# Hevagog/as-cops-and-thieves

Measured on AMD Instinct MI355X. Metric: env-steps/sec (whole node) at 4096 parallel envs, 2v1 agents, 64-ray sensors, higher is better.
Workload: dtype f64; 1 GPU; 2 cops vs 1 thieves, labyrinth map (30 hull walls / 119 planes), 4096 envs per GPU, 64 rays/agent, dt=1/60, max_step_count=400, Philox random actions, auto-reset; envs_per_gpu=4096, rays=64, agents=3, map=labyrinth, parallelism=env-sharded x1, no data-path collective, episodes_reset_per_gpu=32768, burn_in_steps=600

## Files before the change

as_cops_and_thieves_amd/_native.py:

```python
from __future__ import annotations

import ctypes as C
import os
import subprocess
from pathlib import Path

from .config import C_FIELDS_F64, C_FIELDS_I32

PKG = Path(__file__).resolve().parent
ROOT = PKG.parent
LIB_PATH = PKG / "libcat_sim.so"
if os.environ.get("CAT_SIM_LIB"):
    LIB_PATH = Path(os.environ["CAT_SIM_LIB"]).resolve()
SRC = PKG / "csrc" / "cat_sim.hip"


def sources():
    return [SRC, *sorted((PKG / "csrc").glob("cat_sim_*.h")), ROOT / "include" / "cat_sim.h"]
HIPCC_FLAGS = ["--offload-arch=gfx950", "-O3", "-ffp-contract=off", "-fPIC", "-shared"]

OUT_FIELDS = ("obs_distance", "obs_type", "hit_shape", "shared_distance", "shared_type",
              "team_positions", "reward", "terminated", "truncated", "winner")
STATE_FIELDS = ("pos", "vel", "vbias", "tc", "leaf_bb", "wall_shape", "wall_age", "wall_jn",
                "pair_age", "pair_jn", "step_count", "reset_count")
# ... 100 lines not shown
    L.cat_grid_free_host.restype = None
    L.cat_map_wall_bb_depth_host.argtypes = [vp, C.c_size_t, C.c_double]
    L.cat_map_wall_bb_depth_host.restype = i32
    if hasattr(L, "cat_bbtree_host"):
        L.cat_bbtree_host.argtypes = [vp, C.c_size_t, vp, vp, i32, vp, vp]
        L.cat_bbtree_host.restype = i32
    if hasattr(L, "cat_plan_describe_host"):
        L.cat_plan_describe_host.argtypes = [vp, vp, vp, vp, i32, vp, C.c_char_p, C.c_size_t]
        L.cat_plan_describe_host.restype = i32
    if hasattr(L, "cat_debug_tree_counts"):
        L.cat_debug_tree_counts.argtypes = [vp, i32]
        L.cat_debug_tree_counts.restype = i32
    if hasattr(L, "cat_radius_thresholds_host"):
        L.cat_radius_thresholds_host.argtypes = [C.c_double, C.c_double, C.c_double, vp]
        L.cat_radius_thresholds_host.restype = i32
    if hasattr(L, "cat_reward_arith_host"):
        L.cat_reward_arith_host.argtypes = [vp, vp, vp]
        L.cat_reward_arith_host.restype = i32
        L.cat_reward_arith_max.argtypes = [vp]
        L.cat_reward_arith_max.restype = i32
        L.cat_debug_reward_table.argtypes = [vp, vp, vp]
        L.cat_debug_reward_table.restype = i32
    for name in ("cat_create", "cat_destroy", "cat_reset", "cat_reset_done", "cat_step", "cat_step_fused", "cat_rollout_fused", "cat_step_repeat", "cat_get_state",
                 "cat_set_state", "cat_random_actions", "cat_set_seed", "cat_device_errors", "cat_arm_kernel_timing", "cat_num_agents", "cat_num_shapes", "cat_selftest_arith", "cat_debug_grid_lookup"):
        getattr(L, name).restype = i32
    _lib = L
    return L


EXPORTED_SYMBOLS = ("cat_abi_version", "cat_one_tick_kernel", "cat_rollout_kernel", "cat_chunks_per_unit", "cat_last_error", "cat_create", "cat_destroy", "cat_reset",
                    "cat_reset_done", "cat_step", "cat_step_fused", "cat_rollout_fused", "cat_step_repeat", "cat_get_state", "cat_set_state", "cat_random_actions",
                    "cat_set_seed", "cat_device_errors", "cat_arm_kernel_timing", "cat_num_agents", "cat_num_shapes", "cat_selftest_arith", "cat_debug_grid_lookup",
                    "cat_grid_build_host", "cat_grid_lookup_host", "cat_grid_bytes_host", "cat_grid_free_host", "cat_map_wall_bb_depth_host",
                    "cat_bbtree_host", "cat_reward_arith_host", "cat_reward_arith_max", "cat_debug_reward_table", "cat_bind_final_positions",
                    "cat_plan_describe_host", "cat_radius_thresholds_host")
```

as_cops_and_thieves_amd/csrc/cat_sim.hip:

```cpp
#include <hip/hip_runtime.h>
#include <hip/hip_ext.h>

#include <cfloat>
#include <cmath>
#include <cstdarg>
#include <cstdint>
#include <cstdio>
#include <cstdlib>
#include <cstring>
#include <algorithm>
#include <atomic>
#include <thread>
#include <type_traits>
#include <sched.h>
#include <string>
#include <vector>

#include "cat_sim.h"

namespace {
#include "cat_sim_common.h"
#include "cat_sim_reward.h"
#include "cat_sim_geometry.h"
#include "cat_sim_fan.h"
#include "cat_sim_physics.h"
#include "cat_sim_scheduler.h"
}

#include "cat_sim_grid.h"
#include "cat_sim_radius.h"
#include "cat_sim_plan.h"
#include "cat_sim_host.h"
```

as_cops_and_thieves_amd/csrc/cat_sim_common.h:

```cpp

constexpr int kMaxWaves = 16;
constexpr int kLanes = 64;
constexpr int kK = CAT_WALL_CACHE;
constexpr int kBB = 6;
constexpr int kPairF = 20;
constexpr unsigned kBlobMagic = 0x31544143u;

struct MapDesc {
    int S, P, A, n_regions;
    int f64_off;
    int i32_off;
    float cmax;
    int PP;
};

struct GridDesc {
    double x0, y0, inv_cell;
    int nx, ny;
    int off_base, ent_base;
    int coff_base, cent_base;
    int crow_base, span;
    int row_base, span_tick;
};

// ... 27 lines not shown
    char *state;
    int rec_bytes, hot_bytes;
    int maxE, ang_ok, row_words, row_id_bits, row_cnt_mul;
    float ang0, inv_step;
    int lds_map_bytes, lds_env_bytes, lds_union_bytes;
    int wpb;
    int lds_pool_off, pool_mask;
    int grp_rays;
    int item_cap;
    unsigned pool_magic; int pool_shift;
    const double *tree_bb;
    const int *tree_link;
    const int *tree_root;
    int lds_racc_off;
    int lds_o16_off;
};

struct DynDims {
    static constexpr bool kFixed = false;
    static constexpr bool kTree = false;
    static __device__ __forceinline__ int A(const Params &p) { return p.A; }
    static __device__ __forceinline__ int R(const Params &p) { return p.R; }
    static __device__ __forceinline__ int n_cops(const Params &p) { return p.n_cops; }
    static __device__ __forceinline__ int NP(const Params &p) { return p.NP; }
    static __device__ __forceinline__ int rec_bytes(const Params &p) { return p.rec_bytes; }
    static __device__ __forceinline__ int hot_bytes(const Params &p) { return p.hot_bytes; }
};
template <int TA, int TR, int TC> struct FixDims {
    static constexpr bool kFixed = true;
    static constexpr bool kTree = false;
// ... 54 lines not shown
        prev = t;
    }
    __device__ void flush(int lane) { if (lane < 24 && acc[lane]) atomicAdd(&g_phase_cycles[lane], acc[lane]); }
};
#define PHASE(pc, id) (pc).mark(id)
#ifdef CAT_EVENT_COUNTS
#define QCOUNT(id) do { const unsigned long long m_ = __ballot(true); if ((int)__builtin_ctzll(m_) == (int)(threadIdx.x % 64)) { \
    atomicAdd(&g_phase_cycles[id], 1ull); atomicAdd(&g_phase_cycles[(id) + 1], (unsigned long long)__popcll(m_)); } } while (0)
#else
#define QCOUNT(id) do {} while (0)
#endif
#else
#define QCOUNT(id) do {} while (0)
struct PhaseClock { __device__ __forceinline__ void flush(int) {} };
#define PHASE(pc, id) do {} while (0)
#endif

struct LaunchArgs {
    cat_outputs out;
    const int *actions;
    union {
        const unsigned char *mask;
        unsigned short *final_pos;
    };
    const double *positions;
    int use_done_mask;
    int auto_reset;
    unsigned long long synth_tick;
    int T;
    int repeat;
// ... 152 lines not shown
```

as_cops_and_thieves_amd/csrc/cat_sim_fan.h:

```cpp
constexpr int kFeatNear = 63;
constexpr int kItemCap = 128;
constexpr int kPassJ = 8;
constexpr int kFanBytes = 2 * kItemCap * 8 + kItemCap * 2 + kPassJ * kLanes * 2;
constexpr int kGroupRays = 256;

__device__ __forceinline__ void poly_query_feat(const Lds &L, float cmax, bool wall, int sh, double r, double cx, double cy, double ax, double ay,
                                                double bx, double by, double r2, double &alpha, int &feat)
{
    const int fc = wall ? L.fc[sh] : 0, first = fc & 0xFFFF, count = fc >> 16;
    const double rsum = r + r2, rr = rsum * rsum;
    const float axf = (float)ax, ayf = (float)ay;
    const float dxf = (float)(bx - ax), dyf = (float)(by - ay);
    const float len2 = dxf * dxf + dyf * dyf, len = sqrtf(len2);
    const float e1 = 1e-6f * (fabsf(axf) + fabsf(ayf) + cmax + 512.0f);
    const float thr = ((float)rsum + 0.01f) * len * 1.00001f + 0.25f + 64.0f * e1;
    const float s_lo = -((float)rsum + 1.0f) * len, s_hi = len2 + ((float)rsum + 1.0f) * len;
    const bool bevels = rsum > 0.0;
    unsigned pm = 0u, vm = wall ? 0u : 1u;
    const double *pl0 = L.planes + 8 * first;
    {
        typedef float f32x2 __attribute__((ext_vector_type(2)));
        const float *q = L.p32 + kPairF * (wall ? L.fp[sh] : 0);
        const f32x2 ax2 = {axf, axf}, ay2 = {ayf, ayf}, dx2 = {dxf, dxf}, dy2 = {dyf, dyf};
        const f32x2 len3 = {3.0f * len, 3.0f * len}, four = {4.0f, 4.0f};
// ... 1005 lines not shown
```

as_cops_and_thieves_amd/csrc/cat_sim_geometry.h:

```cpp
__device__ __forceinline__ double bb_segment_query(const double *bb, double ax, double ay, double dx,
                                                   double dy, double idx, double idy)
{
    const double2 lo = *reinterpret_cast<const double2 *>(bb);
    const double2 hi = *reinterpret_cast<const double2 *>(bb + 2);
    double tmin = -INFINITY, tmax = INFINITY;
    if (dx == 0.0) {
        if (ax < lo.x || hi.x < ax) return INFINITY;
    } else {
        double t1 = (lo.x - ax) * idx, t2 = (hi.x - ax) * idx;
        tmin = CAT_FMAX(tmin, CAT_FMIN(t1, t2));
        tmax = CAT_FMIN(tmax, CAT_FMAX(t1, t2));
    }
    if (dy == 0.0) {
        if (ay < lo.y || hi.y < ay) return INFINITY;
    } else {
        double t1 = (lo.y - ay) * idy, t2 = (hi.y - ay) * idy;
        tmin = CAT_FMAX(tmin, CAT_FMIN(t1, t2));
        tmax = CAT_FMIN(tmax, CAT_FMAX(t1, t2));
    }
    if (tmin <= tmax && 0.0 <= tmax && tmin <= 1.0) return CAT_FMAX(tmin, 0.0);
    return INFINITY;
}

struct SegInfo { int hit; double alpha, px, py; };

__device__ __forceinline__ void circle_segment_query(double cx, double cy, double r1, double ax, double ay,
                                                     double bx, double by, double r2, SegInfo &info)
{
    double dax = ax - cx, day = ay - cy, dbx = bx - cx, dby = by - cy;
    double rsum = r1 + r2;
    double dada = dax * dax + day * day, dadb = dax * dbx + day * dby, dbdb = dbx * dbx + dby * dby;
    double qa = dada - 2.0 * dadb + dbdb;
    double qb = dadb - dada;
    double det = qb * qb - qa * (dada - rsum * rsum);
// ... 99 lines not shown
```

as_cops_and_thieves_amd/csrc/cat_sim_host.h:

```cpp
struct Part {
    GridHost grid;
    std::vector<int> map_ids;
    Params p;
    Params *dev_p = nullptr;
    Prologue pro;
    int n_blocks = 0, wpb = 0, n_envs = 0;
    size_t lds_bytes = 0;
    bool pool_step = false;
    KernelChoice kernels;
};

struct cat_sim {
    std::vector<Part> parts;
    int device;
    hipStream_t side = nullptr;
    hipEvent_t ev_fork = nullptr, ev_join = nullptr;
    hipEvent_t t_start = nullptr, t_stop = nullptr;
    uint16_t *final_pos = nullptr;
    std::vector<MapDesc> maps;
    std::vector<void *> allocs;
    std::string one_tick_name, rollout_name;
    char err[256];
};

// ... 378 lines not shown
        return CAT_ERR_NO_DEVICE;
    }
    if (hipSetDevice(device) != hipSuccess) return CAT_ERR_NO_DEVICE;
    hipLaunchKernelGGL(selftest_kernel, dim3((n + 255) / 256), dim3(256), 0, static_cast<hipStream_t>(stream), op, a, b, out, n);
    return hipGetLastError() == hipSuccess ? CAT_OK : CAT_ERR_HIP;
}

extern "C" int cat_radius_thresholds_host(double term_radius, double agent_radius, double ray_radius, double *out2)
{
    if (!out2) return CAT_ERR_BAD_ARG;
    out2[0] = radius_lt_threshold(term_radius);
    out2[1] = radius_le_threshold(agent_radius, ray_radius);
    return CAT_OK;
}

extern "C" int cat_reward_arith_host(const float *cop_lut, const float *thief_lut, float *out)
{
    if (out)
        for (int i = 0; i < 2 * 32768; i++) out[i] = (float)ra_host_f16_to_f64(reward_arith_f16(i < 32768, (unsigned)i & 0x7FFFu));
    return cop_lut && thief_lut ? reward_arith_scan(cop_lut, thief_lut) : -1;
}

extern "C" int cat_reward_arith_max(const cat_sim *s)
{
    if (!s) return CAT_ERR_BAD_ARG;
    std::vector<float> lut(2 * 32768);
    if (hipSetDevice(s->device) != hipSuccess) return CAT_ERR_NO_DEVICE;
    if (hipMemcpy(lut.data(), s->parts[0].p.cop_lut, 32768 * sizeof(float), hipMemcpyDeviceToHost) != hipSuccess ||
        hipMemcpy(lut.data() + 32768, s->parts[0].p.thief_lut, 32768 * sizeof(float), hipMemcpyDeviceToHost) != hipSuccess) return CAT_ERR_HIP;
    return reward_arith_scan(lut.data(), lut.data() + 32768);
// ... 10 lines not shown
```

as_cops_and_thieves_amd/csrc/cat_sim_physics.h:

```cpp

__device__ __forceinline__ int circle_poly_contact(const Lds &L, int sh, double rp, double cx, double cy, double rc, int lane,
                                   double &nx, double &ny, double &p1x, double &p1y, double &p2x, double &p2y)
{
    const int fc = uni(L.fc[sh]), first = fc & 0xFFFF, count = fc >> 16;
    double sep = -INFINITY, dd = INFINITY, tt = 0.0, ppx = 0.0, ppy = 0.0;
    if (lane < count) {
        const double *pl = L.planes + 8 * (first + lane);
        sep = pl[0] * (cx - pl[2]) + pl[1] * (cy - pl[3]);
    }
    if (__ballot(sep > rc + rp + 1e-9) != 0ull) return 0;
    if (lane < count) {
        const int i = lane;
        const double *pl = L.planes + 8 * (first + i);
        const double *pv = L.planes + 8 * (first + (i - 1 + count) % count);
        double ax_ = pl[2] - cx, ay_ = pl[3] - cy, bx_ = pv[2] - cx, by_ = pv[3] - cy;
        double dx = bx_ - ax_, dy = by_ - ay_;
        double t = -fmin2(fmax2((dx * (ax_ + bx_) + dy * (ay_ + by_)) / (dx * dx + dy * dy), -1.0), 1.0);
        double ht = 0.5 * t;
        ppx = ax_ * (0.5 - ht) + bx_ * (0.5 + ht); ppy = ay_ * (0.5 - ht) + by_ * (0.5 + ht);
        dd = ppx * ppx + ppy * ppy;
        tt = t;
    }
    const bool inside = __ballot(sep > 0.0) == 0ull;
    int best = 0, sepi = 0;
// ... 254 lines not shown
            else L.wag[lane] = a;
        }
    }
    if (lane < D::NP(p)) {
        const int page = L.pag[lane];
        if (page >= 0 && !((seen_p >> lane) & 1u)) {
            const int a = page + 1;
            if (a >= p.persistence) { L.pag[lane] = -1; L.pjn[lane] = 0.0; }
            else L.pag[lane] = a;
        }
    }
    wave_sync();
    PHASE(pc, 15);
    if (nc == 0) return;
    wave_sync();
    const double m_inv = 1.0 / p.mass;
    const int q = lane;
    const bool own = q < nc;
    {
        int ka = -1, kb = -1;
        if (own) { const int *ci = reinterpret_cast<const int *>(L.conf + kConD * q + 12); ka = ci[0]; kb = ci[1]; }
        bool reg = __ballot(kb >= 0) == 0ull;
        int k0 = 0, kn = 0;
        for (int i = 0; reg && i < A; i++) {
            const unsigned long long mk = __ballot(ka == i);
            if (mk == 0ull) continue;
            const int n_i = __popcll(mk), f_i = __builtin_ctzll(mk);
            if (n_i > kSolveReg || mk != (((1ull << n_i) - 1ull) << f_i)) { reg = false; break; }
            if (lane == i) { k0 = f_i; kn = n_i; }
        }
        if (reg) { solve_walls_reg(L, p, lane, k0, kn, m_inv); wave_sync(); return; }
// ... 59 lines not shown
```

as_cops_and_thieves_amd/csrc/cat_sim_plan.h:

```cpp

struct RecLayout {
    int A, NPs;
    constexpr explicit RecLayout(int a) : A(a), NPs(a * (a - 1) / 2 > 0 ? a * (a - 1) / 2 : 1) {}
    constexpr int pos() const { return 0; }
    constexpr int vel() const { return 16 * A; }
    constexpr int vbias() const { return 32 * A; }
    constexpr int tc() const { return 48 * A; }
    constexpr int leaf_bb() const { return 64 * A; }
    constexpr int step_count() const { return 96 * A; }
    constexpr int reset_count() const { return 96 * A + 4; }
    constexpr int hot_bytes() const { return 96 * A + 16; }
    constexpr int wall_jn() const { return hot_bytes(); }
    constexpr int pair_jn() const { return hot_bytes() + A * kK * 8; }
    constexpr int wall_shape() const { return hot_bytes() + (A * kK + NPs) * 8; }
    constexpr int wall_age() const { return wall_shape() + A * kK * 4; }
    constexpr int pair_age() const { return wall_shape() + 2 * A * kK * 4; }
    constexpr int cold_bytes() const { return ((A * kK + NPs) * 8 + (2 * A * kK + NPs) * 4 + 15) / 16 * 16; }
    constexpr int rec_bytes() const { return hot_bytes() + cold_bytes(); }
};

struct LdsSizes {
    int map, env, uni;
    int racc;
    int o16;
// ... 486 lines not shown
        if (slot_map_ids) plan.slot[e] = slot_map_ids[e];
        if (plan.slot[e] < 0 || plan.slot[e] >= n_maps) PLAN_FAIL(CAT_ERR_BAD_SLOT_MAP, "slot_map_ids[%d]=%d out of range", e, plan.slot[e]);
    }
    std::vector<GridHost> map_grid;
    plan_map_grids(cfg, tab, plan, map_grid);
    Params &base = plan.base;
    memset(&base, 0, sizeof base);
    base.N = N; base.A = A; base.n_cops = cfg->n_cops; base.R = cfg->n_rays; base.max_step = cfg->max_step_count;
    base.iterations = cfg->iterations; base.persistence = cfg->persistence; base.gate = cfg->bbtree_gate;
    base.NP = A * (A - 1) / 2;
    base.env_id_offset = cfg->env_id_offset; base.seed = cfg->seed;
    base.dt = cfg->dt; base.bias_coef = cfg->bias_coef; base.slop = cfg->slop; base.ray_length = cfg->ray_length;
    base.ray_radius = cfg->ray_radius; base.rc = cfg->agent_radius; base.mass = cfg->agent_mass; base.impulse = cfg->impulse;
    base.max_speed = cfg->max_speed; base.term_radius = cfg->termination_radius; base.wall_r = cfg->wall_radius;
    base.term_d2 = radius_lt_threshold(base.term_radius); base.near_d2 = radius_le_threshold(base.rc, base.ray_radius);
    base.hot_bytes = RecLayout(A).hot_bytes();
    base.rec_bytes = RecLayout(A).rec_bytes();
    if (base.hot_bytes > kLanes * 16) PLAN_FAIL(CAT_ERR_BAD_CONFIG, "state record of %d bytes exceeds the kernels' register staging", base.hot_bytes);
    split_parts(cfg, map_grid, plan);
    plan_initial_records(cfg, plan);
    {
        const double two_pi = 6.283185307179586;
        const double a0 = atan2(tab->ray_dy[0], tab->ray_dx[0]);
        const double step = two_pi / base.R;
        bool ok = base.R >= 4;
        for (int k = 0; k < base.R && ok; k++) {
            double d = atan2(tab->ray_dy[k], tab->ray_dx[k]) - (a0 + k * step);
            d -= two_pi * floor(d / two_pi + 0.5);
            if (fabs(d) > 1e-6) ok = false;
        }
// ... 124 lines not shown
```

as_cops_and_thieves_amd/csrc/cat_sim_scheduler.h:

```cpp
template <class D>
__device__ __forceinline__ Lds carve(const Params &p, char *smem, const MapDesc &md, int slot, int wave)
{
    Lds L;
    const int S = md.S, P = md.P, W = p.wpb;
    L.bb = reinterpret_cast<const double *>(smem);
    L.planes = L.bb + kBB * S;
    L.p32 = reinterpret_cast<const float *>(L.planes + 8 * P);
    L.fc = reinterpret_cast<const int *>(L.planes + geo_rest_doubles(md));
    L.fp = L.fc + S;
    L.rayd = reinterpret_cast<const double *>(smem + p.lds_map_bytes - 16 * D::R(p));
    L.ctrl = reinterpret_cast<int *>(smem + p.lds_map_bytes);
    char *w = smem + p.lds_map_bytes + ctrl_bytes(W) + slot * p.lds_env_bytes;
    const int A = D::A(p), R = D::R(p), NPs = D::NP(p) > 0 ? D::NP(p) : 1;
    L.rec = w;
    double *d = reinterpret_cast<double *>(w);
    L.pos = d; d += 2 * A; L.vel = d; d += 2 * A; L.vb = d; d += 2 * A; L.tc = d; d += 2 * A;
    L.leaf = d; d += 4 * A;
    L.cnt = reinterpret_cast<int *>(d);
    d = reinterpret_cast<double *>(w + D::hot_bytes(p));
    L.wjn = d; d += A * kK; L.pjn = d; d += NPs;
    {
        int *ri = reinterpret_cast<int *>(d);
        L.wsh = ri; ri += A * kK; L.wag = ri; ri += A * kK; L.pag = ri;
    }
// ... 370 lines not shown
                                          int env, int row_t, int lane, int act_pref, unsigned long long synth_tick, int n_fan, PhaseClock &pc)
{
    int captured, timeout, step;
    SetupRow row;
    {
        const Params &p = *(const Params *)launder(pk);
        const int S = md.S, A = D::A(p);
        row = setup_row(L.pos, p, gd, lane, A);
        step = uni(L.cnt[0]) + 1;
        captured = termination_captured<D>(L, p, S, lane);
        timeout = (!captured && step >= p.max_step) ? 1 : 0;
        copy_snapshot(L, A, lane);

        if (lane < A) {
            const int i = lane;
            const double m_inv = 1.0 / p.mass;
            int act;
            if (la.actions) act = act_pref;
            else { unsigned rnd[4]; philox_env(p, env, (unsigned)synth_tick, (unsigned)i, 0xAC710u, rnd); act = (int)(rnd[0] & 3u); }
            if ((unsigned)act > 3u) atomicOr(p.err_word, CAT_DEVERR_BAD_ACTION);
            double jx = 0.0, jy = 0.0;
            if (act == 0) jx = -p.impulse; else if (act == 1) jy = p.impulse;
            else if (act == 2) jx = p.impulse; else if (act == 3) jy = -p.impulse;
            double vx = L.vel[2 * i] + jx * m_inv, vy = L.vel[2 * i + 1] + jy * m_inv;
            double len = sqrt(vx * vx + vy * vy);
            if (len > p.max_speed) { vx = vx / len * p.max_speed; vy = vy / len * p.max_speed; }
            L.vel[2 * i] = vx; L.vel[2 * i + 1] = vy;
        }
        wave_sync();
        PHASE(pc, 2);
    }
// ... 223 lines not shown

template <class D>
__global__ __launch_bounds__(kMaxWaves *kLanes) void step_kernel(const Params *__restrict__ pp0, const LaunchArgs la0, const Prologue)
{
    rollout_body<D, true>(pp0, la0);
}

#ifdef CAT_WB_COUNTS
__device__ unsigned long long g_wb_counts[8];
extern "C" int cat_debug_wb_counts(unsigned long long *out8, int reset)
{
    unsigned long long h[8];
    if (hipMemcpyFromSymbol(h, HIP_SYMBOL(g_wb_counts), sizeof h) != hipSuccess) return -1;
    for (int i = 0; i < 8; i++) out8[i] = h[i];
    if (reset) { memset(h, 0, sizeof h); if (hipMemcpyToSymbol(HIP_SYMBOL(g_wb_counts), h, sizeof h) != hipSuccess) return -1; }
    return 0;
}
#endif
template <class T> __device__ __forceinline__ T *slot_ptr(T *p0, int sl, int envb) { return (T *)((char *)const_cast<typename std::remove_const<T>::type *>(p0) + sl * envb); }
constexpr unsigned kPoolValid = 0x80000000u;
constexpr double kPoolEmptyRows = 0.05;
#ifndef CAT_POOL_ROUND
#define CAT_POOL_ROUND 60
#endif
#ifndef CAT_POOL_MIN_PARTIAL
#define CAT_POOL_MIN_PARTIAL 40
#endif
#ifndef CAT_POOL_PATIENCE
#define CAT_POOL_PATIENCE 3
#endif
// ... 108 lines not shown
    return n_res;
}

template <class D, bool kExact, bool kRowGate = false>
__device__ __forceinline__ unsigned pool_round(const Lds &L0, const Params &p, const LaunchArgs &la, int S, float cmax, int base, int n, int lane, int *ctrl,
                               unsigned long long *pool, PhaseClock &pc)
{
    const int A = D::A(p), R = D::R(p), envb = p.lds_env_bytes;
    const double r2 = p.ray_radius;
    const unsigned d_empty = f64_to_f16(p.ray_length);
    const unsigned long long lt_mask = (1ull << lane) - 1ull;
    const int gate = launder(uni(p.gate)), n_cops = launder(uni(D::n_cops(p)));
    const double wall_r = launder(p.wall_r), rc = launder(p.rc);
    const int idb = launder(uni(p.row_id_bits)), cmul = launder(uni(p.row_cnt_mul));
    auto row_count = [&](unsigned w) -> int { return w ? (((31 - __builtin_clz(w)) * cmul) >> 16) + 1 : 0; };
    bool on = lane < n;
    unsigned w0 = 0u, meta = 0u;
    if (on) {
        unsigned long long *e = &pool[ring_pos<kExact>(p, (unsigned)(base + lane))];
        unsigned long long v = 0ull;
        int spins = 0;
        do { v = __hip_atomic_load(e, __ATOMIC_RELAXED, __HIP_MEMORY_SCOPE_WORKGROUP); } while (!(v >> 63) && ++spins < kSpinLimit);
        if (!(v >> 63)) { atomicOr(p.err_word, CAT_DEVERR_SCHEDULER); on = false; }
        __hip_atomic_store(e, 0ull, __ATOMIC_RELAXED, __HIP_MEMORY_SCOPE_WORKGROUP);
        w0 = (unsigned)v; meta = (unsigned)(v >> 32);
    }
    lds_acquire();
    const int s = (int)((meta >> 24) & 15u), i = (int)((meta >> 16) & 7u), k = (int)(meta & 255u);
    const unsigned dynmask = on ? ((meta >> 8) & 255u) : 0u;
    if (!on) w0 = 0u;
    unsigned *const rlist = L0.arow;
    rlist[lane] = meta;
    const double *const fpos = slot_ptr(L0.fpos, s, envb), *const ftc = slot_ptr(L0.ftc, s, envb), *const fleaf = slot_ptr(L0.fleaf, s, envb);
    const double2 org = *reinterpret_cast<const double2 *>(fpos + 2 * i);
    const double ax = org.x, ay = org.y;
    const int cnt_w = row_count(w0);
    const int cnt = cnt_w + __popc(dynmask);
    double rdx, rdy, rix, riy;
    {
        const double bx = ax + L0.rayd[2 * k], by = ay + L0.rayd[2 * k + 1];
        rdx = bx - ax; rdy = by - ay; rix = 1.0 / rdx; riy = 1.0 / rdy;
    }
    double best_a = 1.0;
    int best_fi = -1;
    int jj0 = 0;
    wave_sync();
    PHASE(pc, 20);
    while (__ballot(cnt > jj0) != 0ull) {
        int n_items = 0, jj = jj0;
        for (; jj < jj0 + kPassJ; jj++) {
            const bool has = cnt > jj;
            if (__ballot(has) == 0ull) break;
            int id = 0;
            double tbb = 0.0;
            if (has) {
                if (jj < cnt_w) id = (int)((w0 >> (idb * jj)) & ((1u << idb) - 1u)) - 1;
                else {
                    unsigned dj = dynmask;
                    for (int q = jj - cnt_w; q > 0; q--) dj &= dj - 1;
                    id = S + __builtin_ctz(dj);
                }
                if (gate) tbb = bb_segment_query((id < S) ? (L0.bb + kBB * id) : (fleaf + 4 * (id - S)), ax, ay, rdx, rdy, rix, riy);
            }
            const bool live = has && tbb < best_a;
            const unsigned long long m = __ballot(live);
            const int c = __popcll(m);
            if (n_items + c > kItemCap) break;
            int t = 0xFFFF;
            if (live) {
                t = n_items + __popcll(m & lt_mask);
                L0.itm[t] = (unsigned short)(lane | (id << 6));
                L0.itbb[t] = tbb;
            }
            L0.itemidx[(jj - jj0) * kLanes + lane] = (unsigned short)t;
            n_items += c;
        }
        const int jj1 = jj;
        wave_sync();
        PHASE(pc, 5);
        for (int t0 = 0; t0 < n_items; t0 += kLanes) {
            const int t = t0 + lane;
            if (t < n_items) {
                const int d = L0.itm[t];
                const int il = d & 63, id = (d >> 6) & 63;
                const unsigned m2 = rlist[il];
                const int s2 = (int)((m2 >> 24) & 15u), ia = (int)((m2 >> 16) & 7u), k2 = (int)(m2 & 255u);
                const double *const fpos2 = slot_ptr(L0.fpos, s2, envb), *const ftc2 = slot_ptr(L0.ftc, s2, envb);
                const double2 o2 = *reinterpret_cast<const double2 *>(fpos2 + 2 * ia);
                const double cbx = o2.x + L0.rayd[2 * k2], cby = o2.y + L0.rayd[2 * k2 + 1];
                double alpha = 2.0;
                int feat = 0;
                {
                    const bool wall = id < S;
                    const int j = wall ? 0 : id - S;
                    const int *const an2 = slot_ptr(L0.anear, s2, envb);
                    const bool inside = wall ? (id == an2[2 * ia] || id == an2[2 * ia + 1]) : ((((unsigned)slot_ptr(L0.adn, s2, envb)[ia] >> j) & 1u) != 0u);
                    if (inside) { alpha = 0.0; feat = kFeatNear; }
                    else {
                        int f;
                        poly_query_feat(L0, cmax, wall, wall ? id : 0, wall ? wall_r : rc, ftc2[2 * j], ftc2[2 * j + 1], o2.x, o2.y, cbx, cby, r2, alpha, f);
                        feat = f < 0 ? 0 : f;
                    }
                }
                L0.ialpha[t] = alpha; L0.itm[t] = (unsigned short)((id << 6) | feat);
            }
        }
        wave_sync();
        PHASE(pc, 6);
        for (int q = jj0; q < jj1; q++) {
            const int t = cnt > q ? (int)L0.itemidx[(q - jj0) * kLanes + lane] : 0xFFFF;
            if (t != 0xFFFF) {
                const double al = L0.ialpha[t];
                if (al < best_a && L0.itbb[t] < best_a) { best_a = al; best_fi = L0.itm[t]; }
            }
        }
        wave_sync();
        PHASE(pc, 7);
        jj0 = jj1;
    }
    unsigned d16 = d_empty, ty = CAT_EMPTY;
    int best = -1;
    if (best_fi >= 0) {
        const double bx = ax + L0.rayd[2 * k], by = ay + L0.rayd[2 * k + 1];
        best = best_fi >> 6;
        const int f = best_fi & 63;
        const double t = best_a;
        double px = bx, py = by;
        if (f != kFeatNear) {
            const bool wall = best < S;
            const int fc = wall ? L0.fc[best] : 0, first = fc & 0xFFFF, count = fc >> 16;
            if (wall && f < count) {
                const double2 nn = *reinterpret_cast<const double2 *>(L0.planes + 8 * (first + f));
                px = (ax * (1.0 - t) + bx * t) - nn.x * r2;
                py = (ay * (1.0 - t) + by * t) - nn.y * r2;
            } else {
                double2 v = *reinterpret_cast<const double2 *>(L0.planes + 8 * (first + (wall ? f - count : 0)) + 2);
                if (!wall) { v.x = ftc[2 * (best - S)]; v.y = ftc[2 * (best - S) + 1]; }
                circle_hit_point(v.x, v.y, ax, ay, bx, by, t, r2, px, py);
            }
        }
        d16 = obs_distance_f16(px, py, slot_ptr(L0.o16, s, envb)[i]);
        ty = (best < S) ? CAT_WALL : ((best - S) >= n_cops ? CAT_THIEF : CAT_COP);
    }
    if (on) {
        const int o = i * R + k;
        slot_ptr(L0.od, s, envb)[o] = (unsigned short)d16;
        slot_ptr(L0.ot, s, envb)[o] = (unsigned char)ty;
        if (la.out.hit_shape) {
            const int ep = rw_epoch((unsigned)ctrl[4 * s]);
            long long eo = (long long)(ep - 1) * p.N + ctrl[4 * s + 3];
            if (kRowGate && la.repeat) {
                const int *const fl = slot_ptr(L0.flags, s, envb);
                eo = (ep >= la.T || fl[1] || fl[2]) ? (long long)ctrl[4 * s + 3] : -1ll;
            }
            if (!kRowGate || eo >= 0) la.out.hit_shape[(size_t)eo * A * R + o] = best;
        }
        const unsigned want = i < n_cops ? CAT_THIEF : CAT_COP;
        if (ty == want) __hip_atomic_fetch_min(&slot_ptr(L0.dmin, s, envb)[i], d16, __ATOMIC_RELAXED, __HIP_MEMORY_SCOPE_WORKGROUP);
// ... 66 lines not shown
    for (;;) {
        while (todo) {
            const int lane = opaque_v(lane0);
            const Params &p = *(const Params *)launder((ParamsK)pp0);
            const LaunchArgs &la = *(const LaunchArgs *)launder(lap0);
            int *const ctrl = reinterpret_cast<int *>(smem + p.lds_map_bytes);
            const BlockDesc *const K = block_desc_lds(smem, p, W);
            const int slot = uni(__builtin_ctz(todo));
            todo &= todo - 1;
            SSPREAD(slot, 0);
            const int e_s = uni(ctrl[4 * slot + 3]), t = uni(ctrl[4 * slot + 2]);
            const Lds Ls = carve<D>(p, smem, K->md, slot, wave);
            int ap = 0;
            if (la.actions && lane < D::A(p)) ap = la.actions[((size_t)((!kOneTick && la.repeat) ? 0 : t) * p.N + e_s) * D::A(p) + lane];
            if (lane == 0) ctrl[4 * slot + 1] = 0;
            const int n2 = slot_front<D>(Ls, (ParamsK)pp0, la, K->md, K->gd, e_s, kOneTick ? 0 : t, lane, ap, la.synth_tick + (unsigned long long)t, 0, pc);
            if (n2 == 0) slot_record_early<D>(Ls, p, la, e_s, t, T, !kOneTick && la.repeat != 0, lane);
            lds_release();
            if (lane == 0) __hip_atomic_store((unsigned *)&ctrl[4 * slot], rw_make(t + 1, n2), __ATOMIC_RELAXED, __HIP_MEMORY_SCOPE_WORKGROUP);
            PHASE(pc, 3);
            long long eo = (long long)t * p.N + e_s;
            if (!kOneTick && la.repeat) eo = (t + 1 >= la.T || uni(Ls.flags[1]) || uni(Ls.flags[2])) ? (long long)e_s : -1ll;
            const int n_res = pool_sort<D, kExact, !kOneTick>(Ls, p, la, K->gd, eo, slot, lane, pool_ctl(smem, p, W), reinterpret_cast<unsigned long long *>(smem + p.lds_pool_off));
            lds_release();
            const int add = n_res + (n2 == 0 ? 1 : 0);
            int old = 0;
            if (lane == 0) old = __hip_atomic_fetch_add(&ctrl[4 * slot + 1], add, __ATOMIC_RELAXED, __HIP_MEMORY_SCOPE_WORKGROUP);
            if (add > 0 && uni(old) + add == D::A(p) * D::R(p) + 1) wbm |= 1u << slot;
            hint = slot;
            WSPREAD(2); SSPREAD(slot, 1);
        }
#ifdef CAT_WB_COUNTS
        if (wbm && lane0 == 0) { const int k_ = __popc(wbm); atomicAdd(&g_wb_counts[k_ > 7 ? 7 : k_], 1ull); }
#endif
        while (wbm) {
            const int lane = opaque_v(lane0);
            const Params &p = *(const Params *)launder((ParamsK)pp0);
            const LaunchArgs &la = *(const LaunchArgs *)launder(lap0);
            int *const ctrl = reinterpret_cast<int *>(smem + p.lds_map_bytes);
            const BlockDesc *const K = block_desc_lds(smem, p, W);
            const int slot = uni(__builtin_ctz(wbm));
            wbm &= wbm - 1;
            lds_acquire();
            PHASE(pc, 16);
            SSPREAD(slot, 12);
            const int e_s = uni(ctrl[4 * slot + 3]), t = uni(ctrl[4 * slot + 2]);
            const Lds Ls = carve<D>(p, smem, K->md, slot, wave);
            const bool rep = !kOneTick && la.repeat != 0;
            const long long eo = rep ? (long long)e_s : (long long)t * p.N + e_s;
            const int step2 = uni(Ls.flags[0]), captured2 = uni(Ls.flags[1]), timeout2 = uni(Ls.flags[2]), rcount = uni(Ls.flags[3]);
            const bool last = t + 1 >= T || (rep && (captured2 || timeout2));
            slot_writeback<D>(Ls, p, la, e_s, eo, lane, 1, last, step2, captured2, timeout2, rcount, lut_c, lut_t, pc, rep ? t : -1, true);
            wave_sync();
            SSPREAD(slot, 13);
            if (!last) { if (lane == 0) ctrl[4 * slot + 2] = t + 1; todo |= 1u << slot; }
            else if (lane == 0) __hip_atomic_store((unsigned *)&ctrl[4 * slot], kRwFinished, __ATOMIC_RELAXED, __HIP_MEMORY_SCOPE_WORKGROUP);
        }
        if (todo) continue;
        int base, n, slot = -1;
        {
            const int lane = opaque_v(lane0);
            const Params &p = *(const Params *)launder((ParamsK)pp0);
            int *const ctrl = reinterpret_cast<int *>(smem + p.lds_map_bytes);
            int *const pctl = pool_ctl(smem, p, W);
            unsigned w_l = kRwFinished;
            if (lane < W) w_l = __hip_atomic_load((unsigned *)&ctrl[4 * lane], __ATOMIC_RELAXED, __HIP_MEMORY_SCOPE_WORKGROUP);
            int hd = 0, tl = 0;
// ... 38 lines not shown
            PHASE(pc, 22);
        }
        {
            const int lane = opaque_v(lane0);
            const Params &p = *(const Params *)launder((ParamsK)pp0);
            const LaunchArgs &la = *(const LaunchArgs *)launder(lap0);
            int *const ctrl = reinterpret_cast<int *>(smem + p.lds_map_bytes);
            const BlockDesc *const K = block_desc_lds(smem, p, W);
            if (n > 0) {
                const Lds L0 = carve<D>(p, smem, K->md, 0, wave);
                wbm |= pool_round<D, kExact, !kOneTick>(L0, p, la, uni(K->md.S), K->md.cmax, base, n, lane, ctrl, reinterpret_cast<unsigned long long *>(smem + p.lds_pool_off), pc);
            } else {
                const Lds Ls = carve<D>(p, smem, K->md, slot, wave);
                SSPREAD(slot, 2);
                PHASE(pc, 9);
                physics_env<D>(Ls, p, uni(K->md.S), lane, pc);
                PHASE(pc, 10);
                slot_record_early<D>(Ls, p, la, uni(ctrl[4 * slot + 3]), uni(ctrl[4 * slot + 2]), T, !kOneTick && la.repeat != 0, lane);
                lds_release();
                SSPREAD(slot, 3);
                int old = 0;
                if (lane == 0) old = __hip_atomic_fetch_add(&ctrl[4 * slot + 1], 1, __ATOMIC_RELAXED, __HIP_MEMORY_SCOPE_WORKGROUP);
                if (uni(old) + 1 == D::A(p) * D::R(p) + 1) wbm |= 1u << slot;
            }
            PHASE(pc, 23);
        }
    }
    PHASE(pc, 11);
    WSPREAD(3); WSPREAD(5);
    pc.flush(lane0);
}

template <class D, bool kExact = false>
// ... 174 lines not shown
```

include/cat_sim.h:

```cpp
#ifndef CAT_SIM_H
#define CAT_SIM_H

#include <stddef.h>
#include <stdint.h>

#ifdef __cplusplus
extern "C" {
#endif

#define CAT_ABI_VERSION 1
#define CAT_MAX_AGENTS 8
#define CAT_MAX_RAYS 512
#define CAT_MAX_SHAPES 256
#define CAT_MAX_HULL_EDGES 31
#define CAT_MAX_ROLLOUT_TICKS 65536
#define CAT_WALL_CACHE 8

enum {
    CAT_OK = 0,
    CAT_ERR_BAD_CONFIG = -1,
    CAT_ERR_BAD_MAP = -2,
    CAT_ERR_BAD_SLOT_MAP = -3,
    CAT_ERR_NO_DEVICE = -4,
    CAT_ERR_HIP = -5,
// ... 120 lines not shown
long long cat_grid_bytes_host(const cat_grid_host *grid);
void cat_grid_free_host(cat_grid_host *grid);

int cat_map_wall_bb_depth_host(const void *map_blob, size_t blob_size, double agent_radius);

int cat_bbtree_host(const void *map_blob, size_t blob_size, double *bb_out, int *link_out, int max_nodes, int *root, int *depth);

int cat_plan_describe_host(const cat_config *cfg, const cat_tables *tables, const void *const *map_blobs, const size_t *blob_sizes,
                           int n_maps, const int32_t *slot_map_ids, char *buf, size_t cap);

int cat_selftest_arith(int op, const double *in_a, const double *in_b, double *out, int n, int device,
                       void *stream);

int cat_radius_thresholds_host(double term_radius, double agent_radius, double ray_radius, double *out2);

int cat_reward_arith_host(const float *cop_lut, const float *thief_lut, float *out);
int cat_reward_arith_max(const cat_sim *sim);
int cat_debug_reward_table(const cat_sim *sim, float *out, void *stream);

#ifdef __cplusplus
}
#endif
#endif
```

Before: 143.1 million env-steps/s.

## Keep pool-round item indices in a register word and streamline ray-box tests

Pool-round item indices for each pass are now packed as bytes of one 64-bit register, replacing a per-lane LDS array, which removes LDS stores and loads in the ray pool loop. Dynamic-shape ids are found by peeling bits incrementally instead of rescanning the mask, and a branch-free slab test is used when no ray in the wave is axis-aligned. The hit point is computed through a unified normal path, and the inverse mass is precomputed in the plan. Ablation and counter macros are added but are off by default. The cost is more register pressure, and the reworked arithmetic could change f64 rounding.

```diff
diff --git a/as_cops_and_thieves_amd/_native.py b/as_cops_and_thieves_amd/_native.py
--- a/as_cops_and_thieves_amd/_native.py
+++ b/as_cops_and_thieves_amd/_native.py
@@ -138,6 +138,11 @@
     if hasattr(L, "cat_radius_thresholds_host"):
         L.cat_radius_thresholds_host.argtypes = [C.c_double, C.c_double, C.c_double, vp]
         L.cat_radius_thresholds_host.restype = i32
+    if hasattr(L, "cat_plan_constants_host"):
+        L.cat_plan_constants_host.argtypes = [vp, vp, vp, vp, i32, vp, vp]
+        L.cat_plan_constants_host.restype = i32
+        L.cat_item_word_host.argtypes = [vp, i32, vp, vp]
+        L.cat_item_word_host.restype = i32
     if hasattr(L, "cat_reward_arith_host"):
         L.cat_reward_arith_host.argtypes = [vp, vp, vp]
         L.cat_reward_arith_host.restype = i32
@@ -157,4 +162,4 @@
                     "cat_set_seed", "cat_device_errors", "cat_arm_kernel_timing", "cat_num_agents", "cat_num_shapes", "cat_selftest_arith", "cat_debug_grid_lookup",
                     "cat_grid_build_host", "cat_grid_lookup_host", "cat_grid_bytes_host", "cat_grid_free_host", "cat_map_wall_bb_depth_host",
                     "cat_bbtree_host", "cat_reward_arith_host", "cat_reward_arith_max", "cat_debug_reward_table", "cat_bind_final_positions",
-                    "cat_plan_describe_host", "cat_radius_thresholds_host")
+                    "cat_plan_describe_host", "cat_radius_thresholds_host", "cat_plan_constants_host", "cat_item_word_host")
diff --git a/as_cops_and_thieves_amd/csrc/cat_sim.hip b/as_cops_and_thieves_amd/csrc/cat_sim.hip
--- a/as_cops_and_thieves_amd/csrc/cat_sim.hip
+++ b/as_cops_and_thieves_amd/csrc/cat_sim.hip
@@ -19,6 +19,7 @@
 #include "cat_sim.h"
 
 namespace {
+#include "cat_sim_consts.h"
 #include "cat_sim_common.h"
 #include "cat_sim_reward.h"
 #include "cat_sim_geometry.h"
diff --git a/as_cops_and_thieves_amd/csrc/cat_sim_common.h b/as_cops_and_thieves_amd/csrc/cat_sim_common.h
--- a/as_cops_and_thieves_amd/csrc/cat_sim_common.h
+++ b/as_cops_and_thieves_amd/csrc/cat_sim_common.h
@@ -65,6 +65,7 @@
     const int *tree_root;
     int lds_racc_off;
     int lds_o16_off;
+    double inv_mass;
 };
 
 struct DynDims {
@@ -149,6 +150,14 @@
 #define QCOUNT(id) do {} while (0)
 struct PhaseClock { __device__ __forceinline__ void flush(int) {} };
 #define PHASE(pc, id) do {} while (0)
+#endif
+
+#ifdef CAT_ROUND_COUNTS
+__device__ unsigned long long g_round_counts[8];
+#define RCOUNT(k, n) do { const unsigned long long m_ = __ballot(true); if ((int)__builtin_ctzll(m_) == (int)(threadIdx.x % 64)) \
+    atomicAdd(&g_round_counts[k], (unsigned long long)(n)); } while (0)
+#else
+#define RCOUNT(k, n) do {} while (0)
 #endif
 
 struct LaunchArgs {
diff --git a/as_cops_and_thieves_amd/csrc/cat_sim_consts.h b/as_cops_and_thieves_amd/csrc/cat_sim_consts.h
--- /dev/null
+++ b/as_cops_and_thieves_amd/csrc/cat_sim_consts.h
@@ -0,0 +1,15 @@
+#pragma once
+#include <cstdint>
+
+#if defined(__HIPCC__)
+#define CAT_HD __host__ __device__ __forceinline__
+#else
+#define CAT_HD inline
+#endif
+
+CAT_HD double inverse_mass(double mass) { return 1.0 / mass; }
+
+constexpr unsigned kItemNone = 0xFFu;
+constexpr uint64_t kItemWordEmpty = ~0ull;
+CAT_HD uint64_t item_word_put(uint64_t w, int j, unsigned t) { return w ^ ((uint64_t)(t ^ kItemNone) << (8 * j)); }
+CAT_HD unsigned item_word_get(uint64_t w, int j) { return (unsigned)(w >> (8 * j)) & 0xFFu; }
diff --git a/as_cops_and_thieves_amd/csrc/cat_sim_fan.h b/as_cops_and_thieves_amd/csrc/cat_sim_fan.h
--- a/as_cops_and_thieves_amd/csrc/cat_sim_fan.h
+++ b/as_cops_and_thieves_amd/csrc/cat_sim_fan.h
@@ -2,6 +2,7 @@
 constexpr int kItemCap = 128;
 constexpr int kPassJ = 8;
 constexpr int kFanBytes = 2 * kItemCap * 8 + kItemCap * 2 + kPassJ * kLanes * 2;
+static_assert(kItemCap <= (int)kItemNone && kPassJ <= 8, "pool_round keeps a pass's item indices as eight bytes of one register (cat_sim_consts.h)");
 constexpr int kGroupRays = 256;
 
 __device__ __forceinline__ void poly_query_feat(const Lds &L, float cmax, bool wall, int sh, double r, double cx, double cy, double ax, double ay,
diff --git a/as_cops_and_thieves_amd/csrc/cat_sim_geometry.h b/as_cops_and_thieves_amd/csrc/cat_sim_geometry.h
--- a/as_cops_and_thieves_amd/csrc/cat_sim_geometry.h
+++ b/as_cops_and_thieves_amd/csrc/cat_sim_geometry.h
@@ -18,6 +18,18 @@
         tmin = CAT_FMAX(tmin, CAT_FMIN(t1, t2));
         tmax = CAT_FMIN(tmax, CAT_FMAX(t1, t2));
     }
+    if (tmin <= tmax && 0.0 <= tmax && tmin <= 1.0) return CAT_FMAX(tmin, 0.0);
+    return INFINITY;
+}
+
+__device__ __forceinline__ double bb_segment_query_nz(const double *bb, double ax, double ay, double idx, double idy)
+{
+    const double2 lo = *reinterpret_cast<const double2 *>(bb);
+    const double2 hi = *reinterpret_cast<const double2 *>(bb + 2);
+    const double x1 = (lo.x - ax) * idx, x2 = (hi.x - ax) * idx;
+    const double y1 = (lo.y - ay) * idy, y2 = (hi.y - ay) * idy;
+    const double tmin = CAT_FMAX(CAT_FMIN(x1, x2), CAT_FMIN(y1, y2));
+    const double tmax = CAT_FMIN(CAT_FMAX(x1, x2), CAT_FMAX(y1, y2));
     if (tmin <= tmax && 0.0 <= tmax && tmin <= 1.0) return CAT_FMAX(tmin, 0.0);
     return INFINITY;
 }
diff --git a/as_cops_and_thieves_amd/csrc/cat_sim_host.h b/as_cops_and_thieves_amd/csrc/cat_sim_host.h
--- a/as_cops_and_thieves_amd/csrc/cat_sim_host.h
+++ b/as_cops_and_thieves_amd/csrc/cat_sim_host.h
@@ -416,6 +416,32 @@
     return CAT_OK;
 }
 
+extern "C" int cat_plan_constants_host(const cat_config *cfg, const cat_tables *tab, const void *const *blobs, const size_t *sizes, int n_maps,
+                                       const int32_t *slot_map_ids, double *out1)
+{
+    if (!out1) return CAT_ERR_BAD_ARG;
+    if (const int rc = check_create_args(cfg, tab, blobs, sizes, n_maps, true, g_create_err)) return rc;
+    SimPlan plan;
+    if (const int rc = plan_sim(cfg, tab, blobs, sizes, n_maps, slot_map_ids, plan, g_create_err)) return rc;
+    for (const PartPlan &pt : plan.parts)
+        if (memcmp(&pt.p.inv_mass, &plan.base.inv_mass, sizeof(double)) != 0) return CAT_ERR_BAD_CONFIG;
+    out1[0] = plan.base.inv_mass;
+    return CAT_OK;
+}
+
+extern "C" int cat_item_word_host(const unsigned char *t, int n, unsigned char *back, unsigned long long *word)
+{
+    if (!t || !back || n < 0 || n > 8) return CAT_ERR_BAD_ARG;
+    uint64_t w = kItemWordEmpty;
+    for (int j = 0; j < n; j++) {
+        if (t[j] >= 128 && t[j] != kItemNone) return CAT_ERR_BAD_ARG;
+        w = item_word_put(w, j, t[j]);
+    }
+    for (int j = 0; j < 8; j++) back[j] = (unsigned char)item_word_get(w, j);
+    if (word) *word = w;
+    return CAT_OK;
+}
+
 extern "C" int cat_reward_arith_host(const float *cop_lut, const float *thief_lut, float *out)
 {
     if (out)
diff --git a/as_cops_and_thieves_amd/csrc/cat_sim_physics.h b/as_cops_and_thieves_amd/csrc/cat_sim_physics.h
--- a/as_cops_and_thieves_amd/csrc/cat_sim_physics.h
+++ b/as_cops_and_thieves_amd/csrc/cat_sim_physics.h
@@ -292,7 +292,7 @@
     PHASE(pc, 15);
     if (nc == 0) return;
     wave_sync();
-    const double m_inv = 1.0 / p.mass;
+    const double m_inv = p.inv_mass;
     const int q = lane;
     const bool own = q < nc;
     {
diff --git a/as_cops_and_thieves_amd/csrc/cat_sim_plan.h b/as_cops_and_thieves_amd/csrc/cat_sim_plan.h
--- a/as_cops_and_thieves_amd/csrc/cat_sim_plan.h
+++ b/as_cops_and_thieves_amd/csrc/cat_sim_plan.h
@@ -524,6 +524,7 @@
     base.ray_radius = cfg->ray_radius; base.rc = cfg->agent_radius; base.mass = cfg->agent_mass; base.impulse = cfg->impulse;
     base.max_speed = cfg->max_speed; base.term_radius = cfg->termination_radius; base.wall_r = cfg->wall_radius;
     base.term_d2 = radius_lt_threshold(base.term_radius); base.near_d2 = radius_le_threshold(base.rc, base.ray_radius);
+    base.inv_mass = inverse_mass(base.mass);
     base.hot_bytes = RecLayout(A).hot_bytes();
     base.rec_bytes = RecLayout(A).rec_bytes();
     if (base.hot_bytes > kLanes * 16) PLAN_FAIL(CAT_ERR_BAD_CONFIG, "state record of %d bytes exceeds the kernels' register staging", base.hot_bytes);
diff --git a/as_cops_and_thieves_amd/csrc/cat_sim_scheduler.h b/as_cops_and_thieves_amd/csrc/cat_sim_scheduler.h
--- a/as_cops_and_thieves_amd/csrc/cat_sim_scheduler.h
+++ b/as_cops_and_thieves_amd/csrc/cat_sim_scheduler.h
@@ -408,7 +408,7 @@
 
         if (lane < A) {
             const int i = lane;
-            const double m_inv = 1.0 / p.mass;
+            const double m_inv = p.inv_mass;
             int act;
             if (la.actions) act = act_pref;
             else { unsigned rnd[4]; philox_env(p, env, (unsigned)synth_tick, (unsigned)i, 0xAC710u, rnd); act = (int)(rnd[0] & 3u); }
@@ -662,6 +662,16 @@
     if (hipMemcpyFromSymbol(h, HIP_SYMBOL(g_wb_counts), sizeof h) != hipSuccess) return -1;
     for (int i = 0; i < 8; i++) out8[i] = h[i];
     if (reset) { memset(h, 0, sizeof h); if (hipMemcpyToSymbol(HIP_SYMBOL(g_wb_counts), h, sizeof h) != hipSuccess) return -1; }
+    return 0;
+}
+#endif
+#ifdef CAT_ROUND_COUNTS
+extern "C" int cat_debug_round_counts(unsigned long long *out8, int reset)
+{
+    unsigned long long h[8];
+    if (hipMemcpyFromSymbol(h, HIP_SYMBOL(g_round_counts), sizeof h) != hipSuccess) return -1;
+    for (int i = 0; i < 8; i++) out8[i] = h[i];
+    if (reset) { memset(h, 0, sizeof h); if (hipMemcpyToSymbol(HIP_SYMBOL(g_round_counts), h, sizeof h) != hipSuccess) return -1; }
     return 0;
 }
 #endif
@@ -800,6 +810,7 @@
     const double wall_r = launder(p.wall_r), rc = launder(p.rc);
     const int idb = launder(uni(p.row_id_bits)), cmul = launder(uni(p.row_cnt_mul));
     auto row_count = [&](unsigned w) -> int { return w ? (((31 - __builtin_clz(w)) * cmul) >> 16) + 1 : 0; };
+    RCOUNT(3, 1);
     bool on = lane < n;
     unsigned w0 = 0u, meta = 0u;
     if (on) {
@@ -817,6 +828,9 @@
     if (!on) w0 = 0u;
     unsigned *const rlist = L0.arow;
     rlist[lane] = meta;
+    unsigned d16 = d_empty, ty = CAT_EMPTY;
+    int best = -1;
+#ifndef CAT_ABL_NOROUND
     const double *const fpos = slot_ptr(L0.fpos, s, envb), *const ftc = slot_ptr(L0.ftc, s, envb), *const fleaf = slot_ptr(L0.fleaf, s, envb);
     const double2 org = *reinterpret_cast<const double2 *>(fpos + 2 * i);
     const double ax = org.x, ay = org.y;
@@ -830,41 +844,49 @@
     double best_a = 1.0;
     int best_fi = -1;
     int jj0 = 0;
+    const bool axis_ray = __ballot(rdx == 0.0 || rdy == 0.0) != 0ull;
+    const char *const bb0 = reinterpret_cast<const char *>(L0.bb);
+    const int leaf_off = (int)(reinterpret_cast<const char *>(fleaf) - bb0) - 32 * S;
+    unsigned dj = dynmask;
     wave_sync();
     PHASE(pc, 20);
     while (__ballot(cnt > jj0) != 0ull) {
         int n_items = 0, jj = jj0;
+        unsigned long long iw = kItemWordEmpty;
         for (; jj < jj0 + kPassJ; jj++) {
             const bool has = cnt > jj;
             if (__ballot(has) == 0ull) break;
-            int id = 0;
+            const bool is_wall = jj < cnt_w;
+            const int id = is_wall ? (int)((w0 >> (idb * jj)) & ((1u << idb) - 1u)) - 1 : S + __builtin_ctz(dj | 0x100u);
             double tbb = 0.0;
-            if (has) {
-                if (jj < cnt_w) id = (int)((w0 >> (idb * jj)) & ((1u << idb) - 1u)) - 1;
-                else {
-                    unsigned dj = dynmask;
-                    for (int q = jj - cnt_w; q > 0; q--) dj &= dj - 1;
-                    id = S + __builtin_ctz(dj);
-                }
-                if (gate) tbb = bb_segment_query((id < S) ? (L0.bb + kBB * id) : (fleaf + 4 * (id - S)), ax, ay, rdx, rdy, rix, riy);
+            if (has && gate) {
+                const double *const bb = reinterpret_cast<const double *>(bb0 + (is_wall ? kBB * 8 * id : leaf_off + 32 * id));
+                tbb = axis_ray ? bb_segment_query(bb, ax, ay, rdx, rdy, rix, riy) : bb_segment_query_nz(bb, ax, ay, rix, riy);
             }
             const bool live = has && tbb < best_a;
             const unsigned long long m = __ballot(live);
             const int c = __popcll(m);
             if (n_items + c > kItemCap) break;
-            int t = 0xFFFF;
+            unsigned t = kItemNone;
             if (live) {
-                t = n_items + __popcll(m & lt_mask);
+                t = (unsigned)(n_items + __popcll(m & lt_mask));
                 L0.itm[t] = (unsigned short)(lane | (id << 6));
                 L0.itbb[t] = tbb;
             }
-            L0.itemidx[(jj - jj0) * kLanes + lane] = (unsigned short)t;
+            RCOUNT(0, 1); RCOUNT(1, c);
+            iw = item_word_put(iw, jj - jj0, t);
+            if (has && !is_wall) dj &= dj - 1;
             n_items += c;
         }
         const int jj1 = jj;
         wave_sync();
         PHASE(pc, 5);
+#ifdef CAT_ABL_NOITEM
+        for (int t = lane; t < n_items; t += kLanes) L0.ialpha[t] = 2.0;
+        if (false)
+#endif
         for (int t0 = 0; t0 < n_items; t0 += kLanes) {
+            RCOUNT(2, 1);
             const int t = t0 + lane;
             if (t < n_items) {
                 const int d = L0.itm[t];
@@ -894,8 +916,8 @@
         wave_sync();
         PHASE(pc, 6);
         for (int q = jj0; q < jj1; q++) {
-            const int t = cnt > q ? (int)L0.itemidx[(q - jj0) * kLanes + lane] : 0xFFFF;
-            if (t != 0xFFFF) {
+            const unsigned t = item_word_get(iw, q - jj0);
+            if (t != kItemNone) {
                 const double al = L0.ialpha[t];
                 if (al < best_a && L0.itbb[t] < best_a) { best_a = al; best_fi = L0.itm[t]; }
             }
@@ -904,8 +926,9 @@
         PHASE(pc, 7);
         jj0 = jj1;
     }
-    unsigned d16 = d_empty, ty = CAT_EMPTY;
-    int best = -1;
+#ifdef CAT_ABL_NOHIT
+    best_fi = -1;
+#endif
     if (best_fi >= 0) {
         const double bx = ax + L0.rayd[2 * k], by = ay + L0.rayd[2 * k + 1];
         best = best_fi >> 6;
@@ -915,19 +938,27 @@
         if (f != kFeatNear) {
             const bool wall = best < S;
             const int fc = wall ? L0.fc[best] : 0, first = fc & 0xFFFF, count = fc >> 16;
-            if (wall && f < count) {
-                const double2 nn = *reinterpret_cast<const double2 *>(L0.planes + 8 * (first + f));
-                px = (ax * (1.0 - t) + bx * t) - nn.x * r2;
-                py = (ay * (1.0 - t) + by * t) - nn.y * r2;
-            } else {
+            const double u = 1.0 - t, qx = ax * u + bx * t, qy = ay * u + by * t;
+            double2 nn;
+            RCOUNT(wall && f < count ? 4 : 5, __popcll(__ballot(true)));
+            if (wall && f < count) nn = *reinterpret_cast<const double2 *>(L0.planes + 8 * (first + f));
+            else {
                 double2 v = *reinterpret_cast<const double2 *>(L0.planes + 8 * (first + (wall ? f - count : 0)) + 2);
                 if (!wall) { v.x = ftc[2 * (best - S)]; v.y = ftc[2 * (best - S) + 1]; }
-                circle_hit_point(v.x, v.y, ax, ay, bx, by, t, r2, px, py);
-            }
+                const double dax = ax - v.x, day = ay - v.y, dbx = bx - v.x, dby = by - v.y;
+                const double lx = dax * u + dbx * t, ly = day * u + dby * t;
+                const double inv = 1.0 / (sqrt(lx * lx + ly * ly) + DBL_MIN);
+                nn.x = lx * inv; nn.y = ly * inv;
+            }
+            px = qx - nn.x * r2;
+            py = qy - nn.y * r2;
         }
         d16 = obs_distance_f16(px, py, slot_ptr(L0.o16, s, envb)[i]);
         ty = (best < S) ? CAT_WALL : ((best - S) >= n_cops ? CAT_THIEF : CAT_COP);
     }
+#else
+    (void)r2; (void)lt_mask; (void)gate; (void)wall_r; (void)rc; (void)row_count; (void)w0; (void)dynmask; (void)cmax;
+#endif
     if (on) {
         const int o = i * R + k;
         slot_ptr(L0.od, s, envb)[o] = (unsigned short)d16;
@@ -1024,14 +1055,25 @@
             int ap = 0;
             if (la.actions && lane < D::A(p)) ap = la.actions[((size_t)((!kOneTick && la.repeat) ? 0 : t) * p.N + e_s) * D::A(p) + lane];
             if (lane == 0) ctrl[4 * slot + 1] = 0;
+#ifndef CAT_ABL_NOFRONT
             const int n2 = slot_front<D>(Ls, (ParamsK)pp0, la, K->md, K->gd, e_s, kOneTick ? 0 : t, lane, ap, la.synth_tick + (unsigned long long)t, 0, pc);
+#else
+            const int n2 = 1;
+            if (lane == 0) { Ls.flags[0] = 1; Ls.flags[1] = 0; Ls.flags[2] = 0; Ls.flags[3] = -1; }
+            (void)ap;
+#endif
             if (n2 == 0) slot_record_early<D>(Ls, p, la, e_s, t, T, !kOneTick && la.repeat != 0, lane);
             lds_release();
             if (lane == 0) __hip_atomic_store((unsigned *)&ctrl[4 * slot], rw_make(t + 1, n2), __ATOMIC_RELAXED, __HIP_MEMORY_SCOPE_WORKGROUP);
             PHASE(pc, 3);
             long long eo = (long long)t * p.N + e_s;
             if (!kOneTick && la.repeat) eo = (t + 1 >= la.T || uni(Ls.flags[1]) || uni(Ls.flags[2])) ? (long long)e_s : -1ll;
+#ifndef CAT_ABL_NOSORT
             const int n_res = pool_sort<D, kExact, !kOneTick>(Ls, p, la, K->gd, eo, slot, lane, pool_ctl(smem, p, W), reinterpret_cast<unsigned long long *>(smem + p.lds_pool_off));
+#else
+            const int n_res = D::A(p) * D::R(p);
+            (void)eo;
+#endif
             lds_release();
             const int add = n_res + (n2 == 0 ? 1 : 0);
             int old = 0;
@@ -1060,7 +1102,9 @@
             const long long eo = rep ? (long long)e_s : (long long)t * p.N + e_s;
             const int step2 = uni(Ls.flags[0]), captured2 = uni(Ls.flags[1]), timeout2 = uni(Ls.flags[2]), rcount = uni(Ls.flags[3]);
             const bool last = t + 1 >= T || (rep && (captured2 || timeout2));
+#ifndef CAT_ABL_NOWB
             slot_writeback<D>(Ls, p, la, e_s, eo, lane, 1, last, step2, captured2, timeout2, rcount, lut_c, lut_t, pc, rep ? t : -1, true);
+#endif
             wave_sync();
             SSPREAD(slot, 13);
             if (!last) { if (lane == 0) ctrl[4 * slot + 2] = t + 1; todo |= 1u << slot; }
@@ -1129,9 +1173,13 @@
                 const Lds Ls = carve<D>(p, smem, K->md, slot, wave);
                 SSPREAD(slot, 2);
                 PHASE(pc, 9);
+#ifndef CAT_ABL_NOPHYS
                 physics_env<D>(Ls, p, uni(K->md.S), lane, pc);
+#endif
                 PHASE(pc, 10);
+#ifndef CAT_ABL_NOPHYS
                 slot_record_early<D>(Ls, p, la, uni(ctrl[4 * slot + 3]), uni(ctrl[4 * slot + 2]), T, !kOneTick && la.repeat != 0, lane);
+#endif
                 lds_release();
                 SSPREAD(slot, 3);
                 int old = 0;
diff --git a/include/cat_sim.h b/include/cat_sim.h
--- a/include/cat_sim.h
+++ b/include/cat_sim.h
@@ -158,6 +158,10 @@
 
 int cat_radius_thresholds_host(double term_radius, double agent_radius, double ray_radius, double *out2);
 
+int cat_plan_constants_host(const cat_config *cfg, const cat_tables *tables, const void *const *map_blobs, const size_t *blob_sizes,
+                            int n_maps, const int32_t *slot_map_ids, double *out1);
+int cat_item_word_host(const unsigned char *t, int n, unsigned char *back, unsigned long long *word);
+
 int cat_reward_arith_host(const float *cop_lut, const float *thief_lut, float *out);
 int cat_reward_arith_max(const cat_sim *sim);
 int cat_debug_reward_table(const cat_sim *sim, float *out, void *stream);
```

After: 144.3 million env-steps/s (median of 6 runs). No clear change (+0.9%).
